# redwarp/kmeans-gpu

Hardware: AMD Instinct MI355X
Metric: pixels/sec per Lloyd iteration (8192x8192, k=256) (higher is better)
Workload: dtype f32; 1 GPU; synthetic uniform RGBA 8192x8192 (seed 0x5EED0003), k=256, one Lloyd iteration = update + assign (labels written every iteration) + accumulate; width=8192, height=8192, k=256, collective_backend=none (one rank), collective_ranks=1, label_pass=before the next iteration, update=by the last launch of the assign pass (kmg_lloyd_assign_update)

## Files before the change

### kmeans-gpu_amd/csrc/kmg_lloyd.hip

```cpp

#include <math.h>

#include "kmg_state.h"

static void drop_events(kmg_lloyd *s)
{
    for (ProfEvent &e : s->events) { s->pool.push_back(e.e0); s->pool.push_back(e.e1); }
    s->events.clear();
}

static void destroy_events(kmg_lloyd *s)
{
    drop_events(s);
    for (hipEvent_t e : s->pool) (void)hipEventDestroy(e);
    s->pool.clear();
}

static int side_flush(kmg_lloyd *s, hipStream_t st)
{
    for (int i = 0; i < 2; ++i)
        if (s->lab_pending[i]) {
            HIP_TRY(hipStreamWaitEvent(st, s->ev_lab[i], 0));
            s->lab_pending[i] = false;
        }
// ... 188 lines not shown
        (void)hipGetLastError();
        if (a) (void)hipFree(a);
        p->affine_failed = true;
        return nullptr;
    }
    p->d_sub_affine = a;
    return a;
}

static int tables_from_histogram(kmg_lloyd *s, uint64_t n_pixels, hipStream_t st)
{
    ColourTable &t = s->tab;
    HIP_TRY(launch_cell_aggregates(t.d_hist, s->p->d_lab_table, t.d_agg, t.d_sub_agg, t.d_occ, st));
    HIP_TRY(launch_work_list(t.d_agg, t.d_work, s->k <= 256 ? n_pixels : 0, st));
    HIP_TRY(hipMemcpyAsync(&t.n_hot, t.d_work + kCells + 1, sizeof(uint32_t), hipMemcpyDeviceToHost, st));
    HIP_TRY(hipMemcpyAsync(&t.n_occ, t.d_work, sizeof(uint32_t), hipMemcpyDeviceToHost, st));
    HIP_TRY(hipStreamSynchronize(st));
    if (const char *e = KMG_TOOLS_ENV("KMG_HOT_CELLS")) { if (e[0] == '0') t.n_hot = 0; }
    t.d_work_share = nullptr;
    t.balance_work = nullptr;
    return KMG_OK;
}

static int bind_image_impl(kmg_lloyd *s, const uint8_t *d_rgba, uint64_t n, void *stream, bool want_tie, uint64_t first_index)
{
    if (!s || !d_rgba || n == 0) return fail(KMG_ERR_INVALID_ARGUMENT, "bad bind_image arguments");
    if (s->side) HIP_TRY(hipStreamSynchronize(s->side));
    s->lab_pending[0] = s->lab_pending[1] = false;
    KMG_TRY(check_pixel_count(n));
    HIP_TRY(hipSetDevice(s->p->device));
    KMG_TRY(ensure_bounds(s->p, S(stream)));
    ColourTable &t = s->tab;
    if (!t.d_hist) {
        const size_t sizes[11] = {sizeof(uint32_t) << 24, sizeof(int64_t) * 4ull * kCells, sizeof(int64_t) * 4ull * kSubCells,
                                  (size_t)1 << 21, cube_work_bytes(), cube_masks_bytes(s->k),
                                  sizeof(uint32_t) * kWorkWords, (size_t)(s->k <= 256 ? 1 : 2) << 24, sub_table_bytes(),
                                  sizeof(uint32_t) * (kCells + 1), cube_balance_bytes()};
        size_t need = 0;
        for (size_t b : sizes) need += pad256(b);
        const hipError_t e = block_take(s->p, need, &t.blk, &t.blk_cap);
        if (e != hipSuccess) {
            t.blk = nullptr; t.blk_cap = 0;
            return fail_hip(e, "colour table allocation");
        }
        size_t off = 0;
        t.d_hist = (uint32_t *)carve(t.blk, off, sizes[0]);
        t.d_agg = (int64_t *)carve(t.blk, off, sizes[1]);
// ... 18 lines not shown
    if (t.d_sub_alt) HIP_TRY(hipMemsetAsync(t.d_sub_alt, 0xFF, sub_table_bytes(), S(stream)));
    if (n >= (1ull << 21)) {
        StreamBuf small, elems, keys;
        hipError_t e = small.alloc(s->p, sizeof(uint32_t) * (4 * 1024 + 1), S(stream));
        if (e == hipSuccess) e = elems.alloc(s->p, sizeof(uint16_t) * n, S(stream));
        if (e == hipSuccess && want_tie) e = keys.alloc(s->p, sizeof(uint32_t) * n, S(stream));
        if (e == hipSuccess)
            e = launch_partitioned_histogram((const uint32_t *)d_rgba, n, first_index, (uint32_t *)small.ptr, (uint16_t *)elems.ptr,
                                             (uint32_t *)keys.ptr, t.d_hist, t.d_tie, S(stream));
        if (e != hipSuccess) return fail_hip(e, "histogram");
    } else {
        HIP_TRY(hipMemsetAsync(t.d_hist, 0, sizeof(uint32_t) << 24, S(stream)));
        HIP_TRY(launch_histogram((const uint32_t *)d_rgba, n, t.d_hist, S(stream)));
        if (want_tie) {
            HIP_TRY(hipMemsetAsync(t.d_tie, 0, sizeof(uint32_t) << 24, S(stream)));
            HIP_TRY(launch_tie_keys((const uint32_t *)d_rgba, n, first_index, t.d_tie, S(stream)));
        }
    }
    if (want_tie) {
        t.tie_valid = true;
        t.tie_first = first_index;
    }
    KMG_TRY(tables_from_histogram(s, n, S(stream)));
    if (want_tie) HIP_TRY(launch_init_records(t.d_work, s->p->d_bounds, t.d_init_cells, S(stream)));
    t.rgba = d_rgba;
    t.n = n;
    return KMG_OK;
}

extern "C" int kmg_lloyd_bind_image(kmg_lloyd *s, const uint8_t *d_rgba, uint64_t n, void *stream)
try {
    if (s) KMG_TRY(check_unweighted(s, "bind_image"));
    KMG_TRY(bind_image_impl(s, d_rgba, n, stream, false, 0));
    s->tab.bound_by_caller = true;
    return KMG_OK;
}
KMG_ABI_CATCH

static int prepare_impl(kmg_lloyd *s, const uint8_t *d_rgba, uint64_t n, int want_labels, int *strategy, void *stream, bool caller)
{
    if (!s || !d_rgba || n == 0) return fail(KMG_ERR_INVALID_ARGUMENT, "bad prepare arguments");
    if (s->weighted) {
        if (drop_binding_of(s, d_rgba)) s->tab.tables_valid = false;
        s->tab.bound_by_init = false;
        if (strategy) *strategy = 0;
        return KMG_OK;
    }
    int chosen = 0;
    const bool fresh = s->tab.rgba == d_rgba && s->tab.n == n && s->tab.bound_by_init;
    s->tab.bound_by_init = false;
    const ImageFacts before = {s->tab.n_occ, s->tab.n_hot};
    bool try_table = n <= 0xFFFFFFFFull && table_pays(s->p, n, s->k, want_labels != 0, fresh ? &before : nullptr);
    if (try_table && !fresh && forced_strategy(s->p) == 0) {
        const ImageFacts dense = {kCells, 0u};
        const double label_pass_s = label_seconds(n, s->k, want_labels != 0);
        const bool sure = cube_seconds(s->k, &dense) + label_pass_s + bind_seconds(n) / 16.0 < scan_seconds(n, s->k, false);
        if (!sure) {
            uint32_t *d_probe = reinterpret_cast<uint32_t *>(s->d_nconv) + 1;
            uint32_t h[3] = {0u, 0u, 1u};
            HIP_TRY(launch_sparsity_probe((const uint32_t *)d_rgba, n, d_probe, S(stream)));
            HIP_TRY(hipMemcpyAsync(h, d_probe, sizeof h, hipMemcpyDeviceToHost, S(stream)));
            HIP_TRY(hipStreamSynchronize(S(stream)));
            double M = (double)h[0];
            for (int it = 0; it < 8 && h[0] < h[2]; ++it) M = (double)h[0] / (1.0 - exp(-(double)h[2] / (M > 1.0 ? M : 1.0)));
            const ImageFacts guess = {(uint32_t)(M < (double)kCells ? M : (double)kCells), h[1] * 10u >= h[2] ? 1u : 0u};
            const double table = cube_seconds(s->k, &guess) + label_pass_s + bind_seconds(n) / 16.0;
            try_table = table < scan_seconds(n, s->k, guess.hot != 0u);
            if (log_debug()) fprintf(stderr, "[kmeans_hip] prepare: %u of %u samples' cells, %u in crowded cells -> ~%u occupied%s: %s\n", h[0], h[2], h[1],
                                     guess.occupied, guess.hot ? ", hot" : "", try_table ? "bind" : "per-pixel scan");
        }
    }
    if (try_table) {
        if (!fresh) KMG_TRY(bind_image_impl(s, d_rgba, n, stream, false, 0));
        const ImageFacts facts = {s->tab.n_occ, s->tab.n_hot};
        if (fresh || table_pays(s->p, n, s->k, want_labels != 0, &facts)) {
            s->tab.bound_by_caller = caller;
            chosen = 1;
        } else {
            s->tab.rgba = nullptr;
            if (log_debug()) fprintf(stderr, "[kmeans_hip] prepare: %u occupied cells, %u hot cells -- the per-pixel scan after all\n", facts.occupied, facts.hot);
        }
    } else {
        drop_binding_of(s, d_rgba);
    }
    if (strategy) *strategy = chosen;
    return KMG_OK;
}

extern "C" int kmg_lloyd_prepare(kmg_lloyd *s, const uint8_t *d_rgba, uint64_t n, int want_labels, int *strategy, void *stream)
try {
    return prepare_impl(s, d_rgba, n, want_labels, strategy, stream, true);
}
KMG_ABI_CATCH

extern "C" int kmg_debug_bound_image(kmg_lloyd *s, uint64_t out[2])
try {
// ... 243 lines not shown
    std::vector<Centroid> own;
    Centroid *h = static_cast<Centroid *>(s->h_slot);
    if (!h || sizeof(Centroid) * s->k > kHostSlotBytes) { own.resize(s->k); h = own.data(); }
    HIP_TRY(hipMemcpyAsync(h, s->d_cent, sizeof(Centroid) * s->k, hipMemcpyDeviceToHost, S(stream)));
    HIP_TRY(hipStreamSynchronize(S(stream)));
    for (uint32_t i = 0; i < s->k; ++i) {
        c4[4 * i] = h[i].L; c4[4 * i + 1] = h[i].a; c4[4 * i + 2] = h[i].b; c4[4 * i + 3] = 1.0f;
    }
    return KMG_OK;
}
KMG_ABI_CATCH

static bool init_table_pays(const kmg_processor *p, uint64_t n, uint32_t k, uint32_t n_seeds = 0)
{
    if (const int f = forced_strategy(p)) return f > 0;
    const double N = (double)n, passes = (double)(n_seeds ? k - n_seeds + 1u : k - 1u);
    const double pixels = k >= 32u && !n_seeds ? (0.3 * k + 18.0) * (9.0e-6 + N * 30.0e-12) : passes * (8.0e-6 + N * 7.0e-12);
    const double colours = passes * 0.9e-5 + (passes < 16.0 ? passes : 16.0) * 3.0e-5 +
                           (n >= (1ull << 21) ? 1.5 * bind_seconds(n) : 5.0e-5 + N * 2.0e-10);
    return colours < pixels;
}

static int init_over_colours(kmg_lloyd *s, const uint8_t *d_rgba, uint64_t n, uint64_t first_index, bool *colours,
                             void *stream, uint32_t n_seeds = 0)
{
    *colours = false;
    if (first_index + n > 0xFFFFFFF0ull || !init_table_pays(s->p, n, s->k, n_seeds)) {
        drop_binding_of(s, d_rgba);
        return KMG_OK;
    }
    ColourTable &t = s->tab;
    if (!t.d_tie) {
        const size_t need = pad256(sizeof(uint32_t) << 24) + pad256(sizeof(float) << 24) + pad256(init_scratch_bytes());
        const hipError_t e = block_take(s->p, need, &t.blk_init, &t.blk_init_cap);
        if (e != hipSuccess) {
            t.blk_init = nullptr; t.blk_init_cap = 0;
            return fail_hip(e, "init tables allocation");
        }
        size_t off = 0;
        t.d_tie = (uint32_t *)carve(t.blk_init, off, sizeof(uint32_t) << 24);
        t.d_cdist = (float *)carve(t.blk_init, off, sizeof(float) << 24);
        t.d_init_cells = carve(t.blk_init, off, init_scratch_bytes());
    }
    KMG_TRY(bind_image_impl(s, d_rgba, n, stream, true, first_index));
    t.bound_by_init = true;
    *colours = true;
    return KMG_OK;
}

static int ensure_dist(kmg_lloyd *s, uint64_t n, hipStream_t st)
{
    if (s->dist_cap >= n) return KMG_OK;
    if (s->d_dist) {
        HIP_TRY(hipStreamSynchronize(st));
        HIP_TRY(hipFree(s->d_dist));
        s->d_dist = nullptr; s->dist_cap = 0; s->dist_blk_cap = 0;
    }
    HIP_TRY(block_take(s->p, sizeof(float) * n, (void **)&s->d_dist, &s->dist_blk_cap));
    s->dist_cap = n;
    return KMG_OK;
}

static uint64_t first_pixel(uint32_t w, uint32_t h)
{
    const int32_t x0 = (int32_t)((float)w * 0.5625f);
    const int32_t y0 = (int32_t)((float)h * 0.93359375f);
    return (uint64_t)y0 * w + (uint64_t)x0;
}

template <class Launch, class Count>
static int init_multi_loop(kmg_lloyd *s, hipStream_t st, const char *route, Launch launch_no, Count count_of)
{
    uint32_t have = 1u, launch = 1u, launches = 0u;
    while (have < s->k) {
        const uint32_t chunk = (launch == 1u ? 1u : 0u) + (s->k - have + 2u) / 3u;
        for (uint32_t q = 0; q < chunk; ++q, ++launch) HIP_TRY(launch_no(launch));
        launches += chunk;
        uint32_t *h = s->h_slot ? static_cast<uint32_t *>(s->h_slot) : &have;
        HIP_TRY(hipMemcpyAsync(h, count_of(launch - 1u), sizeof(uint32_t), hipMemcpyDeviceToHost, st));
        HIP_TRY(hipStreamSynchronize(st));
        have = *static_cast<volatile uint32_t *>(h);
        if (have == 0u || have > s->k) return fail(KMG_ERR_HIP, "initialisation: centroid count %u out of range", have);
    }
    if (log_debug()) fprintf(stderr, "[kmeans_hip] initialisation%s: %u centroids in %u launches\n", route, s->k, launches);
    return KMG_OK;
}

static int init_single_picks(kmg_lloyd *s, const uint32_t *rgba, uint64_t n, uint32_t first_j, bool colours, hipStream_t st)
{
    if (colours) {
        for (uint32_t j = first_j; j <= s->k; ++j)
            HIP_TRY(launch_init_pass_cells(s->tab.d_tie, s->tab.d_occ, s->p->d_lab_table, s->d_cent, j, j < s->k ? 1 : 0, s->tab.d_cdist,
                                           s->tab.d_init_cells, nullptr, rgba, s->p->d_lut, st));
        return KMG_OK;
    }
    unsigned long long *slots = (unsigned long long *)s->d_partials;
    for (uint32_t j = first_j; j < s->k; ++j) HIP_TRY(launch_init_pass(rgba, n, s->p->d_lut, s->d_cent, j, s->d_dist, slots, 0, st, true));
    HIP_TRY(launch_init_pick_slots(rgba, n, s->p->d_lut, slots, s->d_cent, s->k - 1u, st));
    return KMG_OK;
}

extern "C" int kmg_lloyd_init_centroids(kmg_lloyd *s, const uint8_t *d_rgba, uint32_t w, uint32_t h, void *stream)
try {
    if (!s || !d_rgba || !w || !h) return fail(KMG_ERR_INVALID_ARGUMENT, "bad init_centroids arguments");
    HIP_TRY(hipSetDevice(s->p->device));
    const uint64_t n = (uint64_t)w * h;
    KMG_TRY(check_pixel_count(n));
    s->tab.tables_valid = false;
    const uint32_t *rgba = (const uint32_t *)d_rgba;
    hipStream_t st = S(stream);
    HIP_TRY(launch_init_first(rgba, first_pixel(w, h), s->p->d_lut, s->d_cent, s->d_key, st));
    if (s->k == 1) { drop_binding_of(s, d_rgba); return KMG_OK; }
    bool colours = false;
    KMG_TRY(init_over_colours(s, d_rgba, n, 0, &colours, stream));
    if (!colours) KMG_TRY(ensure_dist(s, n, st));
    if (!colours && s->k >= 32u && init_multi_bytes(n) <= sizeof(int64_t) * 4ull * s->k * 2048ull)
        return init_multi_loop(s, st, "",
            [&](uint32_t i) { return launch_init_multi(rgba, n, s->p->d_lut, s->d_cent, s->k, i, s->d_dist, s->d_partials, st); },
            [&](uint32_t i) { return init_multi_count(s->d_partials, n, i); });
    if (colours && s->k >= 32u)
        return init_multi_loop(s, st, " over the colours",
            [&](uint32_t i) { return launch_init_cells_multi(s->tab.d_tie, s->tab.d_occ, s->p->d_lab_table, s->d_cent, s->k, i, s->tab.d_cdist,
                                                             s->tab.d_init_cells, rgba, s->p->d_lut, st); },
            [&](uint32_t i) { return init_cells_multi_count(s->tab.d_init_cells, i); });
    return init_single_picks(s, rgba, n, 1u, colours, st);
}
KMG_ABI_CATCH

extern "C" int kmg_lloyd_init_centroids_seeded(kmg_lloyd *s, const uint8_t *d_rgba, uint32_t w, uint32_t h, const float *seeds4,
                                               uint32_t n_seeds, void *stream)
try {
    if (n_seeds == 0) return kmg_lloyd_init_centroids(s, d_rgba, w, h, stream);
    if (!s || !d_rgba || !w || !h || !seeds4) return fail(KMG_ERR_INVALID_ARGUMENT, "bad init_centroids_seeded arguments");
    if (n_seeds > s->k) return fail(KMG_ERR_INVALID_ARGUMENT, "init_centroids_seeded: %u seeds for k = %u", n_seeds, s->k);
    for (uint32_t i = 0; i < 4u * n_seeds; ++i)
        if ((i & 3u) != 3u && !(seeds4[i] - seeds4[i] == 0.0f)) return fail(KMG_ERR_INVALID_ARGUMENT, "init_centroids_seeded: seed %u is not finite", i / 4u);
    HIP_TRY(hipSetDevice(s->p->device));
    const uint64_t n = (uint64_t)w * h;
    KMG_TRY(check_pixel_count(n));
    s->tab.tables_valid = false;
    std::vector<Centroid> seeds(n_seeds);
    for (uint32_t i = 0; i < n_seeds; ++i) seeds[i] = centroid_of(seeds4 + 4 * i);
    HIP_TRY(hipMemcpyAsync(s->d_cent, seeds.data(), sizeof(Centroid) * n_seeds, hipMemcpyHostToDevice, S(stream)));
    HIP_TRY(hipStreamSynchronize(S(stream)));
    if (s->k == n_seeds) {
        drop_binding_of(s, d_rgba);
        return KMG_OK;
// ... 537 lines not shown
```

### kmeans-gpu_amd/csrc/kmg_table.h

```cpp
#pragma once

#include <hip/hip_runtime.h>
#include <stdint.h>

#include "kmg_kernels.h"

namespace kmg {

constexpr uint32_t kCells = 32768;
constexpr uint32_t kCellColours = 512;
constexpr uint32_t kSubCells = kCells * 8;
constexpr uint32_t kCubeGrid = 2048;
constexpr uint32_t kMergeRows = 64;
constexpr uint32_t kHotMax = 56;
constexpr uint32_t kWorkWords = kCells + 1 + 1 + kHotMax;

constexpr uint16_t kSubEmpty = 0xFFFF;
constexpr uint16_t kSubMixed = 0xFFFE;

struct alignas(16) CellBounds {
    float L0, L1, a0, a1, b0, b1, C0, C1, wC0, wC1, wH0, wH1;
    float pad[4];
};

// ... 57 lines not shown
    const int tlo = (int)((e >> 23) & 63u);
    const int w = (int)(e >> 29);
    const int thr = tlo + w + (w == 7 ? 64 : 0);
    if (p < tlo) return e & 255u;
    if (p >= thr) return (e >> 8) & 255u;
    return kPairFine;
}

hipError_t launch_cell_bounds(const float *lut, CellBounds *bounds, CellBounds *sub_bounds, float4 *lab_table, hipStream_t st);
hipError_t launch_histogram(const uint32_t *rgba, uint64_t n, uint32_t *hist, hipStream_t st);
hipError_t launch_partitioned_histogram(const uint32_t *rgba, uint64_t n, uint64_t first_index, uint32_t *small,
                                        uint16_t *elems, uint32_t *keys, uint32_t *hist, uint32_t *tie, hipStream_t st);
hipError_t launch_cell_aggregates(const uint32_t *hist, const float4 *lab_table, int64_t *agg, int64_t *sub_agg, uint8_t *occ_bits,
                                  hipStream_t st);
hipError_t launch_work_list(const int64_t *agg, uint32_t *work, uint64_t n_pixels, hipStream_t st);
hipError_t launch_sparsity_probe(const uint32_t *rgba, uint64_t n, uint32_t *out3, hipStream_t st);
hipError_t launch_work_share(const uint32_t *work, uint32_t part, uint32_t parts, uint32_t *out, hipStream_t st);
hipError_t launch_tie_keys(const uint32_t *rgba, uint64_t n, uint64_t first_index, uint32_t *tie, hipStream_t st);
size_t init_scratch_bytes();
hipError_t launch_init_records(const uint32_t *work, const CellBounds *bounds, void *init_scratch, hipStream_t st);
hipError_t launch_init_pass_cells(const uint32_t *tie, const uint8_t *occ_bits, const float4 *lab_table, Centroid *cent,
                                  uint32_t j, int do_pass, float *dist, void *init_scratch, unsigned long long *band_key,
                                  const uint32_t *pick_rgba, const float *lut, hipStream_t st);
hipError_t launch_init_cells_multi(const uint32_t *tie, const uint8_t *occ_bits, const float4 *lab_table, Centroid *cent, uint32_t k,
                                   uint32_t launch, float *dist, void *init_scratch, const uint32_t *pick_rgba, const float *lut,
                                   hipStream_t st);
const uint32_t *init_cells_multi_count(const void *init_scratch, uint32_t launch);
size_t cube_work_bytes();
constexpr uint32_t kCubeNoEntries = 0x10000u;
constexpr uint32_t kCubeHot = 0x40000u;
constexpr uint32_t kCubeSplitLong = 0x80000u;
constexpr uint32_t kCubeSmallMaxK = 32;
bool cube_single_launch(uint32_t k, uint32_t flags);
hipError_t launch_cube_entries(const uint32_t *work, const uint8_t *occ_bits, const void *colour_labels, uint16_t *sub_table,
                               uint32_t k, hipStream_t st);
struct CubeTail {
    int64_t *acc_out = nullptr;
    int do_update = 0;
    float convergence = 0.0f;
    Centroid *cent = nullptr;
    uint32_t *n_converged = nullptr;
};
struct CubeBalance {
    uint16_t *state = nullptr;
    uint32_t pass = 0;
};
size_t cube_balance_bytes();
struct CubePass {
    const uint32_t *hist = nullptr;
// ... 63 lines not shown
```

### kmeans-gpu_amd/csrc/kmg_table.hip

```cpp

#include "kmg_internal.h"
#include "kmg_table_dev.h"

#include <hip/hip_fp16.h>

namespace kmg {

__global__ __launch_bounds__(kBlock) void k_cell_bounds(const float *__restrict__ lut,
                                                        CellBounds *__restrict__ bounds,
                                                        CellBounds *__restrict__ sub_bounds,
                                                        float4 *__restrict__ lab_table)
{
    __shared__ float s_lut[256];
    __shared__ float s_min[6][8], s_max[6][8];
    s_lut[threadIdx.x] = lut[threadIdx.x];
    __syncthreads();
    const uint32_t wv = threadIdx.x >> 6, lane = threadIdx.x & 63;
#pragma unroll
    for (uint32_t pass = 0; pass < 2u; ++pass) {
        const uint32_t c = pass * kBlock + threadIdx.x;
        float L, a, b;
        colour_to_lab(s_lut, blockIdx.x * kCellColours + c, L, a, b);
        const PixelTerms p = pixel_terms(L, a, b);
        lab_table[blockIdx.x * kCellColours + c] = make_float4(p.L, p.a, p.b, p.C);
// ... 596 lines not shown
        *key = b;
    }
}

hipError_t launch_init_pass_cells(const uint32_t *tie, const uint8_t *occ_bits, const float4 *lab_table, Centroid *cent,
                                  uint32_t j, int do_pass, float *dist, void *init_scratch, unsigned long long *band_key,
                                  const uint32_t *pick_rgba, const float *lut, hipStream_t st)
{
    InitRecord *records = (InitRecord *)init_scratch;
    InitSlot *slots = (InitSlot *)(records + kCells);
    if (band_key) {
        hipLaunchKernelGGL(k_init_fused<false>, dim3(kInitGrid), dim3(kInitBlock), 0, st, tie, occ_bits, lab_table, cent, j, 1,
                           dist, records, slots, pick_rgba, lut);
        hipLaunchKernelGGL(k_init_reduce_slots, dim3(1), dim3(kInitGrid), 0, st, slots, j, band_key);
    } else {
        hipLaunchKernelGGL(k_init_fused<true>, dim3(kInitGrid), dim3(kInitBlock), 0, st, tie, occ_bits, lab_table, cent, j, do_pass,
                           dist, records, slots, pick_rgba, lut);
    }
    return hipGetLastError();
}

constexpr uint32_t kCellMulti = 4;
constexpr uint32_t kCellCands = 8;

struct alignas(16) CellCand {
    unsigned long long key;
    float L, a, b;
    uint32_t box[3];
};
static_assert(sizeof(CellCand) == 32, "CellCand layout");

size_t init_scratch_bytes()
{
    return sizeof(InitRecord) * (size_t)kCells + sizeof(InitSlot) * 2u * kInitGrid + sizeof(CellCand) * 2u * kInitGrid * kCellMulti + 256u;
}

__device__ __forceinline__ uint32_t pack_box(float lo, float hi)
{
    return (uint32_t)__half_as_ushort(__float2half_rd(lo)) | ((uint32_t)__half_as_ushort(__float2half_ru(hi)) << 16);
}

__device__ __forceinline__ float box_far2(const uint32_t *box, float L, float a, float b)
{
    float far[3];
    const float v[3] = {L, a, b};
#pragma unroll
    for (int q = 0; q < 3; ++q) {
        const float lo = __half2float(__ushort_as_half((unsigned short)(box[q] & 0xFFFFu)));
        const float hi = __half2float(__ushort_as_half((unsigned short)(box[q] >> 16)));
        far[q] = fmaxf(fabsf(hi - v[q]), fabsf(v[q] - lo));
    }
    return far[0] * far[0] + far[1] * far[1] + far[2] * far[2];
}

__device__ __forceinline__ CellCand no_cand()
{
    CellCand o; o.key = 0ull; o.L = 0.0f; o.a = 0.0f; o.b = 0.0f; o.box[0] = 0u; o.box[1] = 0u; o.box[2] = 0u;
    return o;
}

__device__ __forceinline__ float lowered_by(float m, const float4 &v, const float4 &c)
{
    const PixelTerms t = pixel_terms_fast(v.x, v.y, v.z, v.w);
    if (!(cie94_key(t, c.x, c.y, c.z, c.w) * (1.0f - 0.0009765625f) > m * m))
        m = fminf(m, cie94_c(v.x, v.y, v.z, v.w, c.x, c.y, c.z, c.w));
    return m;
}

template <int N>
__device__ __forceinline__ unsigned long long init_visit_part_multi(uint32_t cell, uint32_t part, uint32_t lane, bool first,
                                                                    const float4 *s_pick, uint32_t mask,
                                                                    const uint32_t *__restrict__ tie, const uint8_t *__restrict__ occ_bits,
                                                                    const float4 *__restrict__ lab_table, float *__restrict__ dist,
                                                                    float4 &lab_out)
{
    constexpr uint32_t kParts = 8u / N;
    const uint32_t within = part * (kCellColours / kParts) + lane * N;
    const uint32_t base = cell * kCellColours + within;
    const uint32_t occ = ((uint32_t)occ_bits[(uint64_t)cell * 64u + (within >> 3)] >> (within & 7u)) & ((1u << N) - 1u);
    float4 v[N];
#pragma unroll
    for (int q = 0; q < N; ++q) v[q] = lab_table[base + q];
    uint32_t t[N];
    float m[N];
    if (N == 4) {
        const uint4 tt = *reinterpret_cast<const uint4 *>(tie + base);
        t[0] = tt.x; t[1] = tt.y; t[2 % N] = tt.z; t[3 % N] = tt.w;
        float4 d = make_float4(1000000.0f, 1000000.0f, 1000000.0f, 1000000.0f);
        if (!first) d = *reinterpret_cast<const float4 *>(dist + base);
        m[0] = d.x; m[1] = d.y; m[2 % N] = d.z; m[3 % N] = d.w;
    } else {
        const uint2 tt = *reinterpret_cast<const uint2 *>(tie + base);
        t[0] = tt.x; t[1] = tt.y;
        float2 d = make_float2(1000000.0f, 1000000.0f);
        if (!first) d = *reinterpret_cast<const float2 *>(dist + base);
        m[0] = d.x; m[1] = d.y;
    }
    for (uint32_t mm = mask; mm; mm &= mm - 1u) {
        const float4 c = s_pick[__builtin_ctz(mm)];
#pragma unroll
        for (int q = 0; q < N; ++q)
            if ((occ >> q) & 1u) m[q] = lowered_by(m[q], v[q], c);
    }
    uint32_t md = 0u;
#pragma unroll
    for (int q = 0; q < N; ++q)
        if ((occ >> q) & 1u) md = max(md, float_to_bits(m[q]));
    if (occ || first) {
        if (N == 4) *reinterpret_cast<float4 *>(dist + base) = make_float4(m[0], m[1], m[2 % N], m[3 % N]);
        else *reinterpret_cast<float2 *>(dist + base) = make_float2(m[0], m[1]);
    }
    const uint32_t wmd = wave_max_u32(md);
    uint32_t low1 = 0u;
    lab_out = make_float4(0.0f, 0.0f, 0.0f, 0.0f);
    if (occ && md == wmd) {
#pragma unroll
        for (int q = 0; q < N; ++q)
            if (((occ >> q) & 1u) && float_to_bits(m[q]) == wmd && t[q] > low1) { low1 = t[q]; lab_out = v[q]; }
    }
    const uint32_t wlow1 = wave_max_u32(low1);
    return (low1 == wlow1 && low1 != 0u) ? (((unsigned long long)wmd << 32) | (unsigned long long)(wlow1 - 1u)) : 0ull;
}

__global__ __launch_bounds__(kInitBlock) void k_init_cells_multi(const uint32_t *__restrict__ tie, const uint8_t *__restrict__ occ_bits,
                                                                 const float4 *__restrict__ lab_table, Centroid *__restrict__ cent,
                                                                 uint32_t k, uint32_t launch, float *__restrict__ dist,
                                                                 InitRecord *__restrict__ records, CellCand *__restrict__ rows,
                                                                 uint32_t *__restrict__ count, const uint32_t *__restrict__ rgba,
                                                                 const float *__restrict__ lut)
{
    constexpr uint32_t kWaves = kInitBlock / 64, kRowWaves = kInitGrid / 64, kOwn = kWaves * 8;
    __shared__ CellCand s_top[kRowWaves * kCellCands];
    __shared__ CellCand s_best[kCellCands];
    __shared__ unsigned long long s_floor[kRowWaves];
    __shared__ float4 s_pick[kCellMulti];
    __shared__ uint32_t s_npick;
    __shared__ CellCand s_met[kOwn];
    __shared__ uint2 s_list[kOwn];
    __shared__ uint32_t s_count;
    __shared__ unsigned long long s_pkey[kWaves];
    __shared__ float4 s_plab[kWaves];
    const uint32_t lane = threadIdx.x & 63, wv = threadIdx.x >> 6;
    const bool first = launch == 1u;

    const uint32_t slot = wv * 8u + (lane & 7u);
    const bool tester = lane < 8u;
    InitRecord rec;
    rec.key = 0ull; rec.cell = kNoCell;
    if (lane < 8u * kCellMulti) rec = records[slot_work_index(blockIdx.x, slot)];
    if (threadIdx.x == 0) s_count = 0u;

    uint32_t have = 0u;
    if (first) {
        if (threadIdx.x == 0) {
            const Centroid c0 = cent[0];
            s_pick[0] = make_float4(c0.L, c0.a, c0.b, c0.C);
            s_npick = 1u;
            if (blockIdx.x == 0) count[1] = 1u;
        }
    } else {
        const CellCand *prev = rows + (uint64_t)((launch - 1u) & 1u) * kInitGrid * kCellMulti;
        CellCand row[kCellMulti];
#pragma unroll
        for (uint32_t e = 0; e < kCellMulti; ++e) {
            row[e] = no_cand();
            if (threadIdx.x < kInitGrid) row[e] = prev[(uint64_t)threadIdx.x * kCellMulti + e];
        }
        have = count[(launch - 1u) & 1u];
        if (have >= k) {
            if (blockIdx.x == 0 && threadIdx.x == 0) count[launch & 1u] = have;
            return;
        }
        if (wv < kRowWaves) {
            const unsigned long long fl = wave_max_u64(row[kCellMulti - 1].key);
            if (lane == 0u) s_floor[wv] = fl;
#pragma unroll
            for (uint32_t r = 0; r < kCellCands; ++r) {
                const unsigned long long g = wave_max_u64(row[0].key);
                if (g == 0ull) {
                    if (lane == 0u) s_top[wv * kCellCands + r] = no_cand();
                } else if (row[0].key == g) {
                    s_top[wv * kCellCands + r] = row[0];
#pragma unroll
                    for (uint32_t e = 0; e + 1 < kCellMulti; ++e) row[e] = row[e + 1];
                    row[kCellMulti - 1] = no_cand();
                }
            }
        }
        __syncthreads();
        if (threadIdx.x < kRowWaves * kCellCands) {
            const CellCand mine = s_top[threadIdx.x];
            uint32_t rank = 0;
            for (uint32_t q = 0; q < kRowWaves * kCellCands; ++q) {
                const unsigned long long o = s_top[q].key;
                rank += (o > mine.key || (o == mine.key && q < threadIdx.x)) ? 1u : 0u;
            }
            if (rank < kCellCands) s_best[rank] = mine;
        }
        __syncthreads();
        if (wv == 0u) {
            float far2[kCellCands], de[kCellCands];
            {
                const CellCand cx = s_best[lane >> 3], cq = s_best[lane & 7u];
                const float f = box_far2(cx.box, cq.L, cq.a, cq.b);
                const float d = cie94(cq.L, cq.a, cq.b, cx.L, cx.a, cx.b);
#pragma unroll
                for (uint32_t q = 0; q < kCellCands; ++q) {
                    far2[q] = __shfl(f, (int)(((lane & 7u) << 3) | q));
                    de[q] = __shfl(d, (int)(((lane & 7u) << 3) | q));
                }
            }
            unsigned long long floor_key = s_floor[0];
#pragma unroll
            for (uint32_t q = 1; q < kRowWaves; ++q) floor_key = s_floor[q] > floor_key ? s_floor[q] : floor_key;
            const uint32_t room = min(kCellMulti, k - have);
            uint32_t picked = 1u, npick = 1u, order = 0u;
            bool stop = (uint32_t)(s_best[0].key >> 32) == 0u;
#pragma unroll
            for (uint32_t i = 1; i < kCellCands; ++i) {
                const unsigned long long ki = s_best[i].key;
                const float di = __uint_as_float((uint32_t)(ki >> 32));
                if (npick >= room || ki <= floor_key || (uint32_t)(ki >> 32) == 0u) stop = true;
                float m = 3.0e38f;
#pragma unroll
                for (uint32_t q = 0; q < kCellCands; ++q)
                    if ((picked >> q) & 1u) m = fminf(m, far2[q]);
                if (__ballot(lane < i && !(m * 1.01f < di * di)) != 0ull) stop = true;
                const bool lowered = __ballot(lane < kCellCands && ((picked >> lane) & 1u) && !(de[i] >= di)) != 0ull;
                if (!stop && !lowered) { picked |= 1u << i; order |= i << (4u * npick); ++npick; }
            }
            if (lane < npick) {
                const CellCand o = s_best[(order >> (4u * lane)) & 15u];
                float4 v = make_float4(o.L, o.a, o.b, 0.0f);
                if ((uint32_t)(o.key >> 32) == 0u) {
                    const uint32_t px = rgba[0];
                    linear100_to_lab(lut[px & 255u], lut[(px >> 8) & 255u], lut[(px >> 16) & 255u], v.x, v.y, v.z);
                }
                v.w = chroma(v.y, v.z);
                s_pick[lane] = v;
                if (blockIdx.x == 0) { Centroid c; c.L = v.x; c.a = v.y; c.b = v.z; c.C = v.w; cent[have + lane] = c; }
            }
            if (lane == 0u) {
                s_npick = npick;
                if (blockIdx.x == 0) count[launch & 1u] = have + npick;
            }
        }
    }
    __syncthreads();
    const uint32_t npick = s_npick;
    if (have + npick >= k) return;

    {
        bool reached = false;
        const uint32_t r = lane >> 3;
        if (r < npick && rec.cell != kNoCell) {
            reached = true;
            if (!first) {
                const float4 c = s_pick[r];
                reached = cie94_lower_bound(rec.cb, c.x, c.y, c.z, c.w) < __uint_as_float((uint32_t)(rec.key >> 32));
            }
        }
        const unsigned long long hits = __ballot(reached);
        if (tester) {
            CellCand met = no_cand();
            if (rec.cell != kNoCell) {
                const uint32_t mine = (uint32_t)(hits >> lane);
                const uint32_t mask = (mine & 1u) | ((mine >> 7) & 2u) | ((mine >> 14) & 4u) | ((mine >> 21) & 8u);
                met.key = rec.key; met.L = rec.lab.x; met.a = rec.lab.y; met.b = rec.lab.z;
                met.box[0] = pack_box(rec.cb.L0, rec.cb.L1); met.box[1] = pack_box(rec.cb.a0, rec.cb.a1); met.box[2] = pack_box(rec.cb.b0, rec.cb.b1);
                if (mask) s_list[atomicAdd(&s_count, 1u)] = make_uint2(rec.cell, slot | (mask << 8));
            }
            s_met[slot] = met;
        }
    }
    __syncthreads();
    const uint32_t count_ = s_count;
    const bool eager = count_ <= kWaves;

    if (count_ <= 8u) {
        const uint32_t shift = count_ <= 4u ? 2u : 1u;
        const uint32_t my = wv >> shift, part = wv & ((1u << shift) - 1u);
        unsigned long long pk = 0ull;
        float4 pl = make_float4(0.0f, 0.0f, 0.0f, 0.0f);
        if (my < count_) {
            const uint2 e = s_list[my];
            pk = shift == 2u ? init_visit_part_multi<2>(e.x, part, lane, first, s_pick, e.y >> 8, tie, occ_bits, lab_table, dist, pl)
                             : init_visit_part_multi<4>(e.x, part, lane, first, s_pick, e.y >> 8, tie, occ_bits, lab_table, dist, pl);
        }
        if (lane == 0u) s_pkey[wv] = 0ull;
        if (pk != 0ull) { s_pkey[wv] = pk; s_plab[wv] = pl; }
        __syncthreads();
        if (part == 0u && my < count_ && lane == 0u) {
            uint32_t w = wv;
            for (uint32_t q = 1; q < (1u << shift); ++q) if (s_pkey[wv + q] > s_pkey[w]) w = wv + q;
            const unsigned long long key = s_pkey[w];
            const float4 lab = s_plab[w];
            const uint32_t sl = s_list[my].y & 255u;
            InitRecord *r = records + slot_work_index(blockIdx.x, sl);
            r->key = key;
            r->lab = lab;
            s_met[sl].key = key; s_met[sl].L = lab.x; s_met[sl].a = lab.y; s_met[sl].b = lab.z;
        }
    }
    uint32_t idx = count_ <= 8u ? count_ : wv;
    uint2 ent = idx < count_ ? s_list[idx] : make_uint2(0u, 0u);
    uint32_t base = ent.x * kCellColours + lane * 8u;
    uint32_t occ = occ_bits[(uint64_t)ent.x * 64u + lane];
    float4 d0 = make_float4(1000000.0f, 1000000.0f, 1000000.0f, 1000000.0f), d1 = d0;
    if (!first) { d0 = *reinterpret_cast<const float4 *>(dist + base); d1 = *reinterpret_cast<const float4 *>(dist + base + 4); }
    while (idx < count_) {
        float4 v[8];
#pragma unroll
        for (int q = 0; q < 8; ++q) v[q] = lab_table[base + q];
        uint4 t0 = make_uint4(0u, 0u, 0u, 0u), t1 = t0;
        if (eager) { t0 = *reinterpret_cast<const uint4 *>(tie + base); t1 = *reinterpret_cast<const uint4 *>(tie + base + 4); }
        const uint32_t idx_n = idx + kWaves;
        const uint2 ent_n = idx_n < count_ ? s_list[idx_n] : ent;
        const uint32_t base_n = ent_n.x * kCellColours + lane * 8u;
        const uint32_t occ_n = occ_bits[(uint64_t)ent_n.x * 64u + lane];
        float4 d0_n = d0, d1_n = d1;
        if (!first) { d0_n = *reinterpret_cast<const float4 *>(dist + base_n); d1_n = *reinterpret_cast<const float4 *>(dist + base_n + 4); }

        float m[8] = {d0.x, d0.y, d0.z, d0.w, d1.x, d1.y, d1.z, d1.w};
        for (uint32_t mm = ent.y >> 8; mm; mm &= mm - 1u) {
            const float4 c = s_pick[__builtin_ctz(mm)];
#pragma unroll
            for (int q = 0; q < 8; ++q)
                if ((occ >> q) & 1u) m[q] = lowered_by(m[q], v[q], c);
        }
        uint32_t md = 0u;
#pragma unroll
        for (int q = 0; q < 8; ++q)
            if ((occ >> q) & 1u) md = max(md, float_to_bits(m[q]));
        if (occ || first) {
            *reinterpret_cast<float4 *>(dist + base) = make_float4(m[0], m[1], m[2], m[3]);
            *reinterpret_cast<float4 *>(dist + base + 4) = make_float4(m[4], m[5], m[6], m[7]);
        }
        const uint32_t wmd = wave_max_u32(md);
        uint32_t low1 = 0u;
        float4 best_lab = make_float4(0.0f, 0.0f, 0.0f, 0.0f);
        if (occ && md == wmd) {
            if (!eager) { t0 = *reinterpret_cast<const uint4 *>(tie + base); t1 = *reinterpret_cast<const uint4 *>(tie + base + 4); }
            const uint32_t t[8] = {t0.x, t0.y, t0.z, t0.w, t1.x, t1.y, t1.z, t1.w};
#pragma unroll
            for (int q = 0; q < 8; ++q) {
                if (((occ >> q) & 1u) && float_to_bits(m[q]) == wmd && t[q] > low1) { low1 = t[q]; best_lab = v[q]; }
            }
        }
        const uint32_t wlow1 = wave_max_u32(low1);
        if (low1 == wlow1 && low1 != 0u) {
            const unsigned long long key = ((unsigned long long)wmd << 32) | (unsigned long long)(wlow1 - 1u);
            const uint32_t sl = ent.y & 255u;
            InitRecord *r = records + slot_work_index(blockIdx.x, sl);
            r->key = key;
            r->lab = best_lab;
            s_met[sl].key = key; s_met[sl].L = best_lab.x; s_met[sl].a = best_lab.y; s_met[sl].b = best_lab.z;
        }
        idx = idx_n; ent = ent_n; base = base_n; occ = occ_n; d0 = d0_n; d1 = d1_n;
    }
    __syncthreads();
    if (wv < kOwn / 64u) {
        CellCand mine = s_met[threadIdx.x];
#pragma unroll
        for (uint32_t r = 0; r < kCellMulti; ++r) {
            const unsigned long long g = wave_max_u64(mine.key);
            if (g == 0ull) {
                if (lane == 0u) s_top[wv * kCellMulti + r] = no_cand();
            } else if (mine.key == g) {
                s_top[wv * kCellMulti + r] = mine;
                mine.key = 0ull;
            }
        }
    }
    __syncthreads();
    if (threadIdx.x < (kOwn / 64u) * kCellMulti) {
        const CellCand mine = s_top[threadIdx.x];
        uint32_t rank = 0;
#pragma unroll
        for (uint32_t q = 0; q < (kOwn / 64u) * kCellMulti; ++q) {
            const unsigned long long o = s_top[q].key;
            rank += (o > mine.key || (o == mine.key && q < threadIdx.x)) ? 1u : 0u;
        }
        if (rank < kCellMulti) rows[((uint64_t)(launch & 1u) * kInitGrid + blockIdx.x) * kCellMulti + rank] = mine;
    }
}

hipError_t launch_init_cells_multi(const uint32_t *tie, const uint8_t *occ_bits, const float4 *lab_table, Centroid *cent, uint32_t k,
                                   uint32_t launch, float *dist, void *init_scratch, const uint32_t *pick_rgba, const float *lut,
                                   hipStream_t st)
{
    InitRecord *records = (InitRecord *)init_scratch;
    CellCand *rows = (CellCand *)((InitSlot *)(records + kCells) + 2u * kInitGrid);
    uint32_t *count = (uint32_t *)(rows + 2u * kInitGrid * kCellMulti);
    hipLaunchKernelGGL(k_init_cells_multi, dim3(kInitGrid), dim3(kInitBlock), 0, st, tie, occ_bits, lab_table, cent, k, launch, dist,
                       records, rows, count, pick_rgba, lut);
    return hipGetLastError();
}

const uint32_t *init_cells_multi_count(const void *init_scratch, uint32_t launch)
{
    const InitRecord *records = (const InitRecord *)init_scratch;
    const CellCand *rows = (const CellCand *)((const InitSlot *)(records + kCells) + 2u * kInitGrid);
    return (const uint32_t *)(rows + 2u * kInitGrid * kCellMulti) + (launch & 1u);
}

__global__ __launch_bounds__(kBlock) void k_cell_aggregates(const uint32_t *__restrict__ hist,
                                                            const float4 *__restrict__ lab_table,
                                                            int64_t *__restrict__ agg, int64_t *__restrict__ sub_agg,
                                                            uint8_t *__restrict__ occ_bits)
{
    const uint32_t cell = blockIdx.x * (kBlock / 64) + (threadIdx.x >> 6);
    const uint32_t lane = threadIdx.x & 63;
    const uint32_t base = cell * kCellColours + lane * 8;
    const uint4 c0 = *reinterpret_cast<const uint4 *>(hist + base);
    const uint4 c1 = *reinterpret_cast<const uint4 *>(hist + base + 4);
    float4 lab8[8];
#pragma unroll
    for (int q = 0; q < 8; ++q) lab8[q] = lab_table[base + q];
// ... 982 lines not shown
```

Baseline: 306.7 billion pixels/s.

## Skip building tie keys during colour-table init unless a real tie occurs

k-means++ initialisation over the colour table no longer builds the per-colour tie-key table up front when k >= 32. It uses positional keys instead and flags candidates whose distances tie. When a tie is detected, it builds the tie keys lazily and relaunches the selection with them. This removes a memset and a full pixel pass from initialisation, but it only affects init and not the timed Lloyd iteration, at the cost of extra kernel complexity and a possible extra launch.

```diff
diff --git a/kmeans-gpu_amd/csrc/kmg_lloyd.hip b/kmeans-gpu_amd/csrc/kmg_lloyd.hip
--- a/kmeans-gpu_amd/csrc/kmg_lloyd.hip
+++ b/kmeans-gpu_amd/csrc/kmg_lloyd.hip
@@ -234,7 +234,7 @@
     return KMG_OK;
 }
 
-static int bind_image_impl(kmg_lloyd *s, const uint8_t *d_rgba, uint64_t n, void *stream, bool want_tie, uint64_t first_index)
+static int bind_image_impl(kmg_lloyd *s, const uint8_t *d_rgba, uint64_t n, void *stream, bool for_init, bool want_tie, uint64_t first_index)
 {
     if (!s || !d_rgba || n == 0) return fail(KMG_ERR_INVALID_ARGUMENT, "bad bind_image arguments");
     if (s->side) HIP_TRY(hipStreamSynchronize(s->side));
@@ -299,7 +299,7 @@
         t.tie_first = first_index;
     }
     KMG_TRY(tables_from_histogram(s, n, S(stream)));
-    if (want_tie) HIP_TRY(launch_init_records(t.d_work, s->p->d_bounds, t.d_init_cells, S(stream)));
+    if (for_init) HIP_TRY(launch_init_records(t.d_work, s->p->d_bounds, t.d_init_cells, S(stream)));
     t.rgba = d_rgba;
     t.n = n;
     return KMG_OK;
@@ -308,7 +308,7 @@
 extern "C" int kmg_lloyd_bind_image(kmg_lloyd *s, const uint8_t *d_rgba, uint64_t n, void *stream)
 try {
     if (s) KMG_TRY(check_unweighted(s, "bind_image"));
-    KMG_TRY(bind_image_impl(s, d_rgba, n, stream, false, 0));
+    KMG_TRY(bind_image_impl(s, d_rgba, n, stream, false, false, 0));
     s->tab.bound_by_caller = true;
     return KMG_OK;
 }
@@ -348,7 +348,7 @@
         }
     }
     if (try_table) {
-        if (!fresh) KMG_TRY(bind_image_impl(s, d_rgba, n, stream, false, 0));
+        if (!fresh) KMG_TRY(bind_image_impl(s, d_rgba, n, stream, false, false, 0));
         const ImageFacts facts = {s->tab.n_occ, s->tab.n_hot};
         if (fresh || table_pays(s->p, n, s->k, want_labels != 0, &facts)) {
             s->tab.bound_by_caller = caller;
@@ -638,7 +638,7 @@
 }
 
 static int init_over_colours(kmg_lloyd *s, const uint8_t *d_rgba, uint64_t n, uint64_t first_index, bool *colours,
-                             void *stream, uint32_t n_seeds = 0)
+                             void *stream, uint32_t n_seeds = 0, bool want_tie = true)
 {
     *colours = false;
     if (first_index + n > 0xFFFFFFF0ull || !init_table_pays(s->p, n, s->k, n_seeds)) {
@@ -658,9 +658,19 @@
         t.d_cdist = (float *)carve(t.blk_init, off, sizeof(float) << 24);
         t.d_init_cells = carve(t.blk_init, off, init_scratch_bytes());
     }
-    KMG_TRY(bind_image_impl(s, d_rgba, n, stream, true, first_index));
+    KMG_TRY(bind_image_impl(s, d_rgba, n, stream, true, want_tie, first_index));
     t.bound_by_init = true;
     *colours = true;
+    return KMG_OK;
+}
+
+static int build_tie_keys(kmg_lloyd *s, hipStream_t st)
+{
+    ColourTable &t = s->tab;
+    HIP_TRY(hipMemsetAsync(t.d_tie, 0, sizeof(uint32_t) << 24, st));
+    HIP_TRY(launch_tie_keys((const uint32_t *)t.rgba, t.n, 0, t.d_tie, st));
+    t.tie_valid = true;
+    t.tie_first = 0;
     return KMG_OK;
 }
 
@@ -684,10 +694,10 @@
     return (uint64_t)y0 * w + (uint64_t)x0;
 }
 
-template <class Launch, class Count>
-static int init_multi_loop(kmg_lloyd *s, hipStream_t st, const char *route, Launch launch_no, Count count_of)
-{
-    uint32_t have = 1u, launch = 1u, launches = 0u;
+template <class Launch, class Count, class Settle>
+static int init_multi_loop(kmg_lloyd *s, hipStream_t st, const char *route, Launch launch_no, Count count_of, Settle settle)
+{
+    uint32_t have = 1u, launch = 1u, launches = 0u, ties = 0u;
     while (have < s->k) {
         const uint32_t chunk = (launch == 1u ? 1u : 0u) + (s->k - have + 2u) / 3u;
         for (uint32_t q = 0; q < chunk; ++q, ++launch) HIP_TRY(launch_no(launch));
@@ -696,9 +706,16 @@
         HIP_TRY(hipMemcpyAsync(h, count_of(launch - 1u), sizeof(uint32_t), hipMemcpyDeviceToHost, st));
         HIP_TRY(hipStreamSynchronize(st));
         have = *static_cast<volatile uint32_t *>(h);
+        if (have & kInitCellsTie) {
+            have &= ~kInitCellsTie;
+            if (ties++ || have == 0u || have >= s->k) return fail(KMG_ERR_HIP, "initialisation: a tie at %u centroids that the tie keys did not settle", have);
+            KMG_TRY(settle(launch++, have));
+            ++launches;
+        }
         if (have == 0u || have > s->k) return fail(KMG_ERR_HIP, "initialisation: centroid count %u out of range", have);
     }
-    if (log_debug()) fprintf(stderr, "[kmeans_hip] initialisation%s: %u centroids in %u launches\n", route, s->k, launches);
+    if (log_debug()) fprintf(stderr, "[kmeans_hip] initialisation%s: %u centroids in %u launches%s\n", route, s->k, launches,
+                             ties ? ", the tie keys built for a tie between colours" : "");
     return KMG_OK;
 }
 
@@ -728,17 +745,27 @@
     HIP_TRY(launch_init_first(rgba, first_pixel(w, h), s->p->d_lut, s->d_cent, s->d_key, st));
     if (s->k == 1) { drop_binding_of(s, d_rgba); return KMG_OK; }
     bool colours = false;
-    KMG_TRY(init_over_colours(s, d_rgba, n, 0, &colours, stream));
+    KMG_TRY(init_over_colours(s, d_rgba, n, 0, &colours, stream, 0, s->k < 32u));
     if (!colours) KMG_TRY(ensure_dist(s, n, st));
     if (!colours && s->k >= 32u && init_multi_bytes(n) <= sizeof(int64_t) * 4ull * s->k * 2048ull)
         return init_multi_loop(s, st, "",
             [&](uint32_t i) { return launch_init_multi(rgba, n, s->p->d_lut, s->d_cent, s->k, i, s->d_dist, s->d_partials, st); },
-            [&](uint32_t i) { return init_multi_count(s->d_partials, n, i); });
-    if (colours && s->k >= 32u)
+            [&](uint32_t i) { return init_multi_count(s->d_partials, n, i); },
+            [&](uint32_t, uint32_t) { return fail(KMG_ERR_HIP, "initialisation: the passes over the pixels have no ties to settle"); });
+    if (colours && s->k >= 32u) {
+        const uint32_t *tie = nullptr;
         return init_multi_loop(s, st, " over the colours",
-            [&](uint32_t i) { return launch_init_cells_multi(s->tab.d_tie, s->tab.d_occ, s->p->d_lab_table, s->d_cent, s->k, i, s->tab.d_cdist,
+            [&](uint32_t i) { return launch_init_cells_multi(tie, s->tab.d_occ, s->p->d_lab_table, s->d_cent, s->k, i, s->tab.d_cdist,
                                                              s->tab.d_init_cells, rgba, s->p->d_lut, st); },
-            [&](uint32_t i) { return init_cells_multi_count(s->tab.d_init_cells, i); });
+            [&](uint32_t i) { return init_cells_multi_count(s->tab.d_init_cells, i); },
+            [&](uint32_t i, uint32_t have) -> int {
+                KMG_TRY(build_tie_keys(s, st));
+                tie = s->tab.d_tie;
+                HIP_TRY(launch_init_cells_multi(tie, s->tab.d_occ, s->p->d_lab_table, s->d_cent, s->k, i, s->tab.d_cdist,
+                                                s->tab.d_init_cells, rgba, s->p->d_lut, st, have));
+                return KMG_OK;
+            });
+    }
     return init_single_picks(s, rgba, n, 1u, colours, st);
 }
 KMG_ABI_CATCH
diff --git a/kmeans-gpu_amd/csrc/kmg_table.h b/kmeans-gpu_amd/csrc/kmg_table.h
--- a/kmeans-gpu_amd/csrc/kmg_table.h
+++ b/kmeans-gpu_amd/csrc/kmg_table.h
@@ -103,9 +103,10 @@
 hipError_t launch_init_pass_cells(const uint32_t *tie, const uint8_t *occ_bits, const float4 *lab_table, Centroid *cent,
                                   uint32_t j, int do_pass, float *dist, void *init_scratch, unsigned long long *band_key,
                                   const uint32_t *pick_rgba, const float *lut, hipStream_t st);
+constexpr uint32_t kInitCellsTie = 0x80000000u;
 hipError_t launch_init_cells_multi(const uint32_t *tie, const uint8_t *occ_bits, const float4 *lab_table, Centroid *cent, uint32_t k,
                                    uint32_t launch, float *dist, void *init_scratch, const uint32_t *pick_rgba, const float *lut,
-                                   hipStream_t st);
+                                   hipStream_t st, uint32_t rekey_have = 0);
 const uint32_t *init_cells_multi_count(const void *init_scratch, uint32_t launch);
 size_t cube_work_bytes();
 constexpr uint32_t kCubeNoEntries = 0x10000u;
diff --git a/kmeans-gpu_amd/csrc/kmg_table.hip b/kmeans-gpu_amd/csrc/kmg_table.hip
--- a/kmeans-gpu_amd/csrc/kmg_table.hip
+++ b/kmeans-gpu_amd/csrc/kmg_table.hip
@@ -642,6 +642,7 @@
 
 constexpr uint32_t kCellMulti = 4;
 constexpr uint32_t kCellCands = 8;
+constexpr uint32_t kInitTie = kInitCellsTie;
 
 struct alignas(16) CellCand {
     unsigned long long key;
@@ -687,6 +688,13 @@
     return m;
 }
 
+constexpr uint32_t kTiedBit = 0x80000000u;
+__device__ __forceinline__ uint32_t keyless_low(uint32_t wlow1, uint32_t holders)
+{
+    const bool several = __ballot(holders > 1u) != 0ull || __popcll(__ballot(holders != 0u)) > 1;
+    return wlow1 | (several ? kTiedBit : 0u);
+}
+
 template <int N>
 __device__ __forceinline__ unsigned long long init_visit_part_multi(uint32_t cell, uint32_t part, uint32_t lane, bool first,
                                                                     const float4 *s_pick, uint32_t mask,
@@ -701,17 +709,24 @@
     float4 v[N];
 #pragma unroll
     for (int q = 0; q < N; ++q) v[q] = lab_table[base + q];
+    const bool keyless = tie == nullptr;
     uint32_t t[N];
     float m[N];
+#pragma unroll
+    for (int q = 0; q < N; ++q) t[q] = base + (uint32_t)q + 1u;
     if (N == 4) {
-        const uint4 tt = *reinterpret_cast<const uint4 *>(tie + base);
-        t[0] = tt.x; t[1] = tt.y; t[2 % N] = tt.z; t[3 % N] = tt.w;
+        if (!keyless) {
+            const uint4 tt = *reinterpret_cast<const uint4 *>(tie + base);
+            t[0] = tt.x; t[1] = tt.y; t[2 % N] = tt.z; t[3 % N] = tt.w;
+        }
         float4 d = make_float4(1000000.0f, 1000000.0f, 1000000.0f, 1000000.0f);
         if (!first) d = *reinterpret_cast<const float4 *>(dist + base);
         m[0] = d.x; m[1] = d.y; m[2 % N] = d.z; m[3 % N] = d.w;
     } else {
-        const uint2 tt = *reinterpret_cast<const uint2 *>(tie + base);
-        t[0] = tt.x; t[1] = tt.y;
+        if (!keyless) {
+            const uint2 tt = *reinterpret_cast<const uint2 *>(tie + base);
+            t[0] = tt.x; t[1] = tt.y;
+        }
         float2 d = make_float2(1000000.0f, 1000000.0f);
         if (!first) d = *reinterpret_cast<const float2 *>(dist + base);
         m[0] = d.x; m[1] = d.y;
@@ -731,15 +746,20 @@
         else *reinterpret_cast<float2 *>(dist + base) = make_float2(m[0], m[1]);
     }
     const uint32_t wmd = wave_max_u32(md);
-    uint32_t low1 = 0u;
+    uint32_t low1 = 0u, holders = 0u;
     lab_out = make_float4(0.0f, 0.0f, 0.0f, 0.0f);
     if (occ && md == wmd) {
 #pragma unroll
-        for (int q = 0; q < N; ++q)
-            if (((occ >> q) & 1u) && float_to_bits(m[q]) == wmd && t[q] > low1) { low1 = t[q]; lab_out = v[q]; }
+        for (int q = 0; q < N; ++q) {
+            if (((occ >> q) & 1u) && float_to_bits(m[q]) == wmd) {
+                ++holders;
+                if (t[q] > low1) { low1 = t[q]; lab_out = v[q]; }
+            }
+        }
     }
     const uint32_t wlow1 = wave_max_u32(low1);
-    return (low1 == wlow1 && low1 != 0u) ? (((unsigned long long)wmd << 32) | (unsigned long long)(wlow1 - 1u)) : 0ull;
+    const uint32_t low = keyless ? keyless_low(wlow1, holders) : wlow1 - 1u;
+    return (low1 == wlow1 && low1 != 0u) ? (((unsigned long long)wmd << 32) | (unsigned long long)low) : 0ull;
 }
 
 __global__ __launch_bounds__(kInitBlock) void k_init_cells_multi(const uint32_t *__restrict__ tie, const uint8_t *__restrict__ occ_bits,
@@ -747,11 +767,14 @@
                                                                  uint32_t k, uint32_t launch, float *__restrict__ dist,
                                                                  InitRecord *__restrict__ records, CellCand *__restrict__ rows,
                                                                  uint32_t *__restrict__ count, const uint32_t *__restrict__ rgba,
-                                                                 const float *__restrict__ lut)
+                                                                 const float *__restrict__ lut, uint32_t rekey_have)
 {
     constexpr uint32_t kWaves = kInitBlock / 64, kRowWaves = kInitGrid / 64, kOwn = kWaves * 8;
+    const bool keyless = tie == nullptr;
+    const bool rekey = rekey_have != 0u;
     __shared__ CellCand s_top[kRowWaves * kCellCands];
-    __shared__ CellCand s_best[kCellCands];
+    __shared__ CellCand s_best[kCellCands + 1];
+    __shared__ uint32_t s_short;
     __shared__ unsigned long long s_floor[kRowWaves];
     __shared__ float4 s_pick[kCellMulti];
     __shared__ uint32_t s_npick;
@@ -768,7 +791,7 @@
     InitRecord rec;
     rec.key = 0ull; rec.cell = kNoCell;
     if (lane < 8u * kCellMulti) rec = records[slot_work_index(blockIdx.x, slot)];
-    if (threadIdx.x == 0) s_count = 0u;
+    if (threadIdx.x == 0) { s_count = 0u; s_short = 0u; }
 
     uint32_t have = 0u;
     if (first) {
@@ -778,6 +801,12 @@
             s_npick = 1u;
             if (blockIdx.x == 0) count[1] = 1u;
         }
+    } else if (rekey) {
+        have = rekey_have;
+        if (threadIdx.x == 0) {
+            s_npick = 0u;
+            if (blockIdx.x == 0) count[launch & 1u] = have;
+        }
     } else {
         const CellCand *prev = rows + (uint64_t)((launch - 1u) & 1u) * kInitGrid * kCellMulti;
         CellCand row[kCellMulti];
@@ -815,7 +844,8 @@
                 const unsigned long long o = s_top[q].key;
                 rank += (o > mine.key || (o == mine.key && q < threadIdx.x)) ? 1u : 0u;
             }
-            if (rank < kCellCands) s_best[rank] = mine;
+            if (rank <= kCellCands) s_best[rank] = mine;
+            if (rank < kCellCands && threadIdx.x % kCellCands == kCellCands - 1u) s_short = 1u;
         }
         __syncthreads();
         if (wv == 0u) {
@@ -834,40 +864,53 @@
 #pragma unroll
             for (uint32_t q = 1; q < kRowWaves; ++q) floor_key = s_floor[q] > floor_key ? s_floor[q] : floor_key;
             const uint32_t room = min(kCellMulti, k - have);
-            uint32_t picked = 1u, npick = 1u, order = 0u;
-            bool stop = (uint32_t)(s_best[0].key >> 32) == 0u;
-#pragma unroll
-            for (uint32_t i = 1; i < kCellCands; ++i) {
-                const unsigned long long ki = s_best[i].key;
-                const float di = __uint_as_float((uint32_t)(ki >> 32));
-                if (npick >= room || ki <= floor_key || (uint32_t)(ki >> 32) == 0u) stop = true;
-                float m = 3.0e38f;
-#pragma unroll
-                for (uint32_t q = 0; q < kCellCands; ++q)
-                    if ((picked >> q) & 1u) m = fminf(m, far2[q]);
-                if (__ballot(lane < i && !(m * 1.01f < di * di)) != 0ull) stop = true;
-                const bool lowered = __ballot(lane < kCellCands && ((picked >> lane) & 1u) && !(de[i] >= di)) != 0ull;
-                if (!stop && !lowered) { picked |= 1u << i; order |= i << (4u * npick); ++npick; }
-            }
-            if (lane < npick) {
-                const CellCand o = s_best[(order >> (4u * lane)) & 15u];
-                float4 v = make_float4(o.L, o.a, o.b, 0.0f);
-                if ((uint32_t)(o.key >> 32) == 0u) {
-                    const uint32_t px = rgba[0];
-                    linear100_to_lab(lut[px & 255u], lut[(px >> 8) & 255u], lut[(px >> 16) & 255u], v.x, v.y, v.z);
+            const uint32_t floor_hi = (uint32_t)(floor_key >> 32);
+            const uint32_t hi0 = (uint32_t)(s_best[0].key >> 32);
+            if (keyless && hi0 != 0u && (((uint32_t)s_best[0].key & kTiedBit) != 0u || (uint32_t)(s_best[1].key >> 32) == hi0 || floor_hi == hi0)) {
+                if (lane == 0u) {
+                    s_npick = kInitTie;
+                    if (blockIdx.x == 0) count[launch & 1u] = have | kInitTie;
                 }
-                v.w = chroma(v.y, v.z);
-                s_pick[lane] = v;
-                if (blockIdx.x == 0) { Centroid c; c.L = v.x; c.a = v.y; c.b = v.z; c.C = v.w; cent[have + lane] = c; }
-            }
-            if (lane == 0u) {
-                s_npick = npick;
-                if (blockIdx.x == 0) count[launch & 1u] = have + npick;
+            } else {
+                uint32_t picked = 1u, npick = 1u, order = 0u;
+                bool stop = hi0 == 0u;
+#pragma unroll
+                for (uint32_t i = 1; i < kCellCands; ++i) {
+                    const unsigned long long ki = s_best[i].key;
+                    const float di = __uint_as_float((uint32_t)(ki >> 32));
+                    if (npick >= room || ki <= floor_key || (uint32_t)(ki >> 32) == 0u) stop = true;
+                    if (keyless && (((uint32_t)ki & kTiedBit) != 0u || (uint32_t)(ki >> 32) == floor_hi ||
+                                    (i + 1u == kCellCands && s_short != 0u) || (uint32_t)(s_best[i + 1u].key >> 32) == (uint32_t)(ki >> 32)))
+                        stop = true;
+                    float m = 3.0e38f;
+#pragma unroll
+                    for (uint32_t q = 0; q < kCellCands; ++q)
+                        if ((picked >> q) & 1u) m = fminf(m, far2[q]);
+                    if (__ballot(lane < i && !(m * 1.01f < di * di)) != 0ull) stop = true;
+                    const bool lowered = __ballot(lane < kCellCands && ((picked >> lane) & 1u) && !(de[i] >= di)) != 0ull;
+                    if (!stop && !lowered) { picked |= 1u << i; order |= i << (4u * npick); ++npick; }
+                }
+                if (lane < npick) {
+                    const CellCand o = s_best[(order >> (4u * lane)) & 15u];
+                    float4 v = make_float4(o.L, o.a, o.b, 0.0f);
+                    if ((uint32_t)(o.key >> 32) == 0u) {
+                        const uint32_t px = rgba[0];
+                        linear100_to_lab(lut[px & 255u], lut[(px >> 8) & 255u], lut[(px >> 16) & 255u], v.x, v.y, v.z);
+                    }
+                    v.w = chroma(v.y, v.z);
+                    s_pick[lane] = v;
+                    if (blockIdx.x == 0) { Centroid c; c.L = v.x; c.a = v.y; c.b = v.z; c.C = v.w; cent[have + lane] = c; }
+                }
+                if (lane == 0u) {
+                    s_npick = npick;
+                    if (blockIdx.x == 0) count[launch & 1u] = have + npick;
+                }
             }
         }
     }
     __syncthreads();
     const uint32_t npick = s_npick;
+    if (npick == kInitTie) return;
     if (have + npick >= k) return;
 
     {
@@ -888,7 +931,7 @@
                 const uint32_t mask = (mine & 1u) | ((mine >> 7) & 2u) | ((mine >> 14) & 4u) | ((mine >> 21) & 8u);
                 met.key = rec.key; met.L = rec.lab.x; met.a = rec.lab.y; met.b = rec.lab.z;
                 met.box[0] = pack_box(rec.cb.L0, rec.cb.L1); met.box[1] = pack_box(rec.cb.a0, rec.cb.a1); met.box[2] = pack_box(rec.cb.b0, rec.cb.b1);
-                if (mask) s_list[atomicAdd(&s_count, 1u)] = make_uint2(rec.cell, slot | (mask << 8));
+                if (mask || rekey) s_list[atomicAdd(&s_count, 1u)] = make_uint2(rec.cell, slot | (mask << 8));
             }
             s_met[slot] = met;
         }
@@ -913,7 +956,10 @@
         if (part == 0u && my < count_ && lane == 0u) {
             uint32_t w = wv;
             for (uint32_t q = 1; q < (1u << shift); ++q) if (s_pkey[wv + q] > s_pkey[w]) w = wv + q;
-            const unsigned long long key = s_pkey[w];
+            unsigned long long key = s_pkey[w];
+            if (keyless)
+                for (uint32_t q = 0; q < (1u << shift); ++q)
+                    if (wv + q != w && s_pkey[wv + q] != 0ull && (uint32_t)(s_pkey[wv + q] >> 32) == (uint32_t)(key >> 32)) key |= kTiedBit;
             const float4 lab = s_plab[w];
             const uint32_t sl = s_list[my].y & 255u;
             InitRecord *r = records + slot_work_index(blockIdx.x, sl);
@@ -933,7 +979,7 @@
 #pragma unroll
         for (int q = 0; q < 8; ++q) v[q] = lab_table[base + q];
         uint4 t0 = make_uint4(0u, 0u, 0u, 0u), t1 = t0;
-        if (eager) { t0 = *reinterpret_cast<const uint4 *>(tie + base); t1 = *reinterpret_cast<const uint4 *>(tie + base + 4); }
+        if (eager && !keyless) { t0 = *reinterpret_cast<const uint4 *>(tie + base); t1 = *reinterpret_cast<const uint4 *>(tie + base + 4); }
         const uint32_t idx_n = idx + kWaves;
         const uint2 ent_n = idx_n < count_ ? s_list[idx_n] : ent;
         const uint32_t base_n = ent_n.x * kCellColours + lane * 8u;
@@ -957,19 +1003,24 @@
             *reinterpret_cast<float4 *>(dist + base + 4) = make_float4(m[4], m[5], m[6], m[7]);
         }
         const uint32_t wmd = wave_max_u32(md);
-        uint32_t low1 = 0u;
+        uint32_t low1 = 0u, holders = 0u;
         float4 best_lab = make_float4(0.0f, 0.0f, 0.0f, 0.0f);
         if (occ && md == wmd) {
-            if (!eager) { t0 = *reinterpret_cast<const uint4 *>(tie + base); t1 = *reinterpret_cast<const uint4 *>(tie + base + 4); }
+            if (!eager && !keyless) { t0 = *reinterpret_cast<const uint4 *>(tie + base); t1 = *reinterpret_cast<const uint4 *>(tie + base + 4); }
             const uint32_t t[8] = {t0.x, t0.y, t0.z, t0.w, t1.x, t1.y, t1.z, t1.w};
 #pragma unroll
             for (int q = 0; q < 8; ++q) {
-                if (((occ >> q) & 1u) && float_to_bits(m[q]) == wmd && t[q] > low1) { low1 = t[q]; best_lab = v[q]; }
+                if (((occ >> q) & 1u) && float_to_bits(m[q]) == wmd) {
+                    const uint32_t tq = keyless ? base + (uint32_t)q + 1u : t[q];
+                    ++holders;
+                    if (tq > low1) { low1 = tq; best_lab = v[q]; }
+                }
             }
         }
         const uint32_t wlow1 = wave_max_u32(low1);
+        const uint32_t low = keyless ? keyless_low(wlow1, holders) : wlow1 - 1u;
         if (low1 == wlow1 && low1 != 0u) {
-            const unsigned long long key = ((unsigned long long)wmd << 32) | (unsigned long long)(wlow1 - 1u);
+            const unsigned long long key = ((unsigned long long)wmd << 32) | (unsigned long long)low;
             const uint32_t sl = ent.y & 255u;
             InitRecord *r = records + slot_work_index(blockIdx.x, sl);
             r->key = key;
@@ -1007,13 +1058,13 @@
 
 hipError_t launch_init_cells_multi(const uint32_t *tie, const uint8_t *occ_bits, const float4 *lab_table, Centroid *cent, uint32_t k,
                                    uint32_t launch, float *dist, void *init_scratch, const uint32_t *pick_rgba, const float *lut,
-                                   hipStream_t st)
+                                   hipStream_t st, uint32_t rekey_have)
 {
     InitRecord *records = (InitRecord *)init_scratch;
     CellCand *rows = (CellCand *)((InitSlot *)(records + kCells) + 2u * kInitGrid);
     uint32_t *count = (uint32_t *)(rows + 2u * kInitGrid * kCellMulti);
     hipLaunchKernelGGL(k_init_cells_multi, dim3(kInitGrid), dim3(kInitBlock), 0, st, tie, occ_bits, lab_table, cent, k, launch, dist,
-                       records, rows, count, pick_rgba, lut);
+                       records, rows, count, pick_rgba, lut, rekey_have);
     return hipGetLastError();
 }
 
```

After: 307.4 billion pixels/s (median of 4 runs). No clear change (+0.2%).
